# drzhn/UnitySimpleRaytracing

Measured on AMD Instinct MI355X. Metric: LBVH build Mtri/s + primary Mrays/s at 1080p on 1M-tri synthetic mesh, higher is better.
Workload: dtype f32+u32; 1 GPU; cfg2: 1,000,000-triangle tiled bumpy torus (seed 2), 1920x1080 primary rays, camera (0,0,250) fov 60; full LBVH rebuild + frame trace per step; triangles=1000000, rays=2073600, trace_mode=fast

## Files before the change

### unitysimpleraytracing_amd/csrc/lbvh_build.hip

```cpp
#include "lbvh_common.h"

namespace {

struct box3 { float mn[3]; float mx[3]; };

__device__ __forceinline__ uint32_t expand_bits(uint32_t v)
{
    v = (v * 0x00010001u) & 0xFF0000FFu;
    v = (v * 0x00000101u) & 0x0F00F00Fu;
    v = (v * 0x00000011u) & 0xC30C30C3u;
    v = (v * 0x00000005u) & 0x49249249u;
    return v;
}

__device__ __forceinline__ uint32_t quantize(float x)
{
    x = fminf(fmaxf(x * 1024.0f, 0.0f), 1023.0f);
    return (uint32_t)x;
}

struct node_reset { uint32_t* internal; uint32_t* leaf; };
__device__ __forceinline__ void reset_node_slot(const node_reset& r, uint32_t i, uint32_t n, uint32_t capacity)
{
    if (!r.internal || i >= capacity) return;
// ... 288 lines not shown

template <typename Pred>
__device__ __forceinline__ uint32_t last_true_64ary(uint32_t lo, uint32_t hi, Pred pred)
{
    const uint32_t lane = lane_id();
    while (hi - lo > 1u) {
        const uint32_t span = hi - lo;
        const uint32_t step = (span + 63u) / 64u;
        const uint32_t l = lo + (lane + 1u) * step;
        const bool p = lane < 63u && l < hi && pred(l);
        const uint64_t m = __ballot(p);
        const uint32_t cnt = (uint32_t)__builtin_ctzll(~m);
        lo += cnt * step;
        hi = min(hi, lo + step);
    }
    return lo;
}

__device__ __forceinline__ void wide_node_range(const uint32_t* __restrict__ codes, int num, int idx, uint32_t self, int d, int dmin,
                                                int& first, int& last)
{
    const uint32_t lane = lane_id();
    auto dlt = [&](int y) -> int { return (y >= 0 && y <= num - 1) ? clz32(self ^ codes[y]) : -1; };
    uint32_t lmax;
    {
        const uint32_t cand = 2u << (lane & 31u);
        const bool p = lane < 31u && dlt(idx + (int)(cand * (uint32_t)d)) > dmin;
        const uint64_t m = __ballot(p);
        lmax = 2u << (uint32_t)__builtin_ctzll(~m);
    }
    const uint32_t l = last_true_64ary(0u, lmax, [&](uint32_t q) { return dlt(idx + (int)(q * (uint32_t)d)) > dmin; });
    const int j = idx + (int)l * d;
    first = min(idx, j);
    last = max(idx, j);
}

__device__ __forceinline__ int wide_node_split(const uint32_t* __restrict__ codes, int first, int last, uint32_t first_code,
                                               uint32_t last_code)
{
    if (first_code == last_code) return (first + last) >> 1;
    const int common_prefix = clz32(first_code ^ last_code);
    return (int)last_true_64ary((uint32_t)first, (uint32_t)last,
                                [&](uint32_t q) { return clz32(first_code ^ codes[q]) > common_prefix; });
}

constexpr int kTreeWords = kTreeWindow / 32;
constexpr int kBitStride = 33;
constexpr int kBitWords = (kTreeWords + 2) * kBitStride;
constexpr int kBitSums = 34;
static_assert(kTreeHalo >= 1 && kTreeWords == (kTreeThreads + 2 * kTreeHalo) / 32 && kTreeWords <= 32,
              "the window of kTreeThreads + 2 * kTreeHalo keys needs a halo, and one 32-bit summary word per B[v]: at most 1024 keys");

template <int J>
__device__ __forceinline__ uint32_t swizzle_xor(uint32_t x)
{
    return (uint32_t)__builtin_amdgcn_ds_swizzle((int)x, (J << 10) | 0x1F);
}

template <int S>
__device__ __forceinline__ uint32_t transpose_step(uint32_t x, uint32_t keep, uint32_t amt)
{
    constexpr uint32_t J = 1u << S;
    const uint32_t y = S == 0   ? (uint32_t)__builtin_amdgcn_update_dpp(0, (int)x, 0xB1, 0xf, 0xf, true)
                       : S == 1 ? (uint32_t)__builtin_amdgcn_update_dpp(0, (int)x, 0x4E, 0xf, 0xf, true)
                                : swizzle_xor<(int)J>(x);
    const uint32_t moved = __builtin_amdgcn_alignbit(y, y, amt);
    return (x & keep) | (moved & ~keep);
}

struct transpose_consts { uint32_t keep[5], amt[5]; };
__device__ __forceinline__ transpose_consts make_transpose_consts(uint32_t lane)
{
    transpose_consts c;
    const uint32_t M[5] = {0x55555555u, 0x33333333u, 0x0F0F0F0Fu, 0x00FF00FFu, 0x0000FFFFu};
#pragma unroll
    for (int s = 0; s < 5; s++) {
        const bool upper = (lane >> s) & 1u;
        c.keep[s] = upper ? ~M[s] : M[s];
        c.amt[s] = upper ? (1u << s) : 32u - (1u << s);
    }
    return c;
}

__device__ __forceinline__ uint32_t transpose32_lanes(uint32_t x, const transpose_consts& c)
{
    x = transpose_step<0>(x, c.keep[0], c.amt[0]);
    x = transpose_step<1>(x, c.keep[1], c.amt[1]);
    x = transpose_step<2>(x, c.keep[2], c.amt[2]);
    x = transpose_step<3>(x, c.keep[3], c.amt[3]);
    x = transpose_step<4>(x, c.keep[4], c.amt[4]);
    return x;
}

typedef __attribute__((address_space(3))) uint32_t lds_u32_rw;
struct delta_bitmaps {
    lds_u32* bits;
    lds_u32* sums;
    __device__ __forceinline__ uint32_t word(int q, int v) const { return bits[(q + 1) * kBitStride + v]; }
    __device__ __forceinline__ bool first_from(int v, int s, int& pos) const
    {
        const int q = s >> 5;
        const u64 w = (((u64)word(q + 1, v) << 32) | word(q, v)) >> (s & 31);
        if (w) { pos = s + __builtin_ctzll(w); return true; }
        const uint32_t rest = sums[v] & ~((4u << q) - 1u);
        if (!rest) return false;
        const int c = __builtin_ctz(rest);
        pos = c * 32 + __builtin_ctz(word(c, v));
        return true;
    }
    __device__ __forceinline__ bool last_upto(int v, int e, int& pos) const
    {
        if (e < 0) return false;
        const int q = e >> 5;
        const u64 w = (((u64)word(q, v) << 32) | word(q - 1, v)) << (31 - (e & 31));
        if (w) { pos = e - __builtin_clzll(w); return true; }
        const uint32_t rest = q >= 1 ? sums[v] & ((1u << (q - 1)) - 1u) : 0u;
        if (!rest) return false;
        const int c = 31 - __builtin_clz(rest);
        pos = c * 32 + 31 - __builtin_clz(word(c, v));
        return true;
    }
};

__device__ __forceinline__ void clear_delta_bitmaps(uint32_t* s_bits, uint32_t* s_sums)
{
    const uint32_t t = threadIdx.x;
    if (t < (uint32_t)kBitStride) s_bits[t] = 0u;
    else if (t < 2u * kBitStride) s_bits[(kTreeWords + 1) * kBitStride + (t - kBitStride)] = 0u;
    else if (t < 2u * kBitStride + kBitSums) s_sums[t - 2u * kBitStride] = 0u;
}

__device__ __forceinline__ void stage_keys_and_bitmaps(const uint32_t* __restrict__ codes, uint32_t* s_keys, uint32_t* s_bits,
                                                       uint32_t* s_sums, const key_window& win)
{
    const uint32_t lane = lane_id(), wave = threadIdx.x >> 6;
    constexpr int kChunks = kTreeWindow / 64, kWaves = kTreeThreads / 64, kPer = kChunks / kWaves;
    static_assert(kChunks % kWaves == 0, "every wave takes the same number of chunks");
    uint32_t key[kPer], next[kPer];
#pragma unroll
    for (int k = 0; k < kPer; k++) {
        const int m = win.w0 + ((int)wave + k * kWaves) * 64 + (int)lane;
        key[k] = m < win.w1 ? codes[m] : 0u;
        next[k] = 0u;
        if (lane == 63u && m + 1 < win.w1) next[k] = codes[m + 1];
    }
    const transpose_consts tc = make_transpose_consts(lane);
    uint32_t some = 0u;
#pragma unroll
    for (int k = 0; k < kPer; k++) {
        const int c = (int)wave + k * kWaves;
        const int p = c * 64 + (int)lane, m = win.w0 + p;
        if (m < win.w1) s_keys[p] = key[k];
        const uint32_t from_next_lane = (uint32_t)__builtin_amdgcn_update_dpp(0, (int)key[k], 0x130, 0xf, 0xf, false);
        const uint32_t nxt = lane == 63u ? next[k] : from_next_lane;
        uint32_t row = 0u;
        if (m + 1 < win.w1) {
            const uint32_t x = key[k] ^ nxt;
            row = x ? 0xFFFFFFFFu << __builtin_clz(x) : 0u;
            if (!x) s_sums[32] = 1u;
        } else if (m + 1 == win.num && m < win.w1) {
            row = 0xFFFFFFFFu;
        }
        const uint32_t x = transpose32_lanes(row, tc);
        const int wd = 2 * c + (int)(lane >> 5);
        s_bits[(wd + 1) * kBitStride + (int)(lane & 31u)] = x;
        some |= x ? 1u << wd : 0u;
    }
    if (some) atomicOr(&s_sums[lane & 31u], some);
}

typedef float f3 __attribute__((ext_vector_type(3)));
struct corner3 { float x, y, z; };
struct hier_t {
    corner3* lo;
    corner3* hi;
    uint32_t n2x2;
    uint32_t levels;
};

__device__ __forceinline__ uint32_t hier_offset(uint32_t n2x2, uint32_t k) { return n2x2 - (n2x2 >> k); }

__device__ __forceinline__ f3 load_corner(const corner3* p) { return *reinterpret_cast<const f3 __attribute__((aligned(4)))*>(p); }
__device__ __forceinline__ void store_corner(corner3* p, float x, float y, float z)
{
    f3 v = {x, y, z};
    *reinterpret_cast<f3 __attribute__((aligned(4)))*>(p) = v;
}

__device__ __forceinline__ void wave_union(float mn[3], float mx[3])
{
#pragma unroll
    for (int d = 1; d < 64; d <<= 1) {
#pragma unroll
        for (int k = 0; k < 3; k++) {
            mn[k] = fminf(mn[k], __shfl_xor(mn[k], d));
            mx[k] = fmaxf(mx[k], __shfl_xor(mx[k], d));
        }
    }
}

typedef uint32_t u3v __attribute__((ext_vector_type(3)));
template <int NQ, int LV, bool BUF>
__device__ __forceinline__ void range_boxes_impl(const hier_t& h, const uint32_t a[NQ], const uint32_t b[NQ], float mn[NQ][3],
                                                 float mx[NQ][3])
{
    const uint32_t neutral = h.n2x2 - 1u;
    __amdgpu_buffer_rsrc_t lo_rsrc, hi_rsrc;
    if (BUF) {
        lo_rsrc = __builtin_amdgcn_make_buffer_rsrc(h.lo, 0, (int)(h.n2x2 * 12u), 0x00020000);
        hi_rsrc = __builtin_amdgcn_make_buffer_rsrc(h.hi, 0, (int)(h.n2x2 * 12u), 0x00020000);
    }
    uint32_t l[NQ], r[NQ];
    bool more = false;
    f3 lo[NQ][LV][2], hi[NQ][LV][2];
#pragma unroll
    for (int q = 0; q < NQ; q++) {
        l[q] = a[q];
        r[q] = b[q] + 1u;
        more = more || l[q] < r[q];
#pragma unroll
        for (int d = 0; d < 3; d++) { mn[q][d] = INFINITY; mx[q][d] = -INFINITY; }
#pragma unroll
        for (int v = 0; v < LV; v++)
#pragma unroll
            for (int e = 0; e < 2; e++) {
                const f3 pinf = {INFINITY, INFINITY, INFINITY}, ninf = {-INFINITY, -INFINITY, -INFINITY};
                lo[q][v][e] = pinf;
                hi[q][v][e] = ninf;
            }
    }
    for (uint32_t k = 0; more; k += LV) {
        uint32_t idx[NQ][LV][2];
        more = false;
#pragma unroll
        for (int v = 0; v < LV; v++) {
            const uint32_t lev = min(k + (uint32_t)v, 31u);
            const uint32_t off = hier_offset(h.n2x2, lev);
#pragma unroll
            for (int q = 0; q < NQ; q++) {
                const bool tl = l[q] < r[q] && (l[q] & 1u);
                idx[q][v][0] = tl ? off + l[q] : neutral;
                l[q] += tl ? 1u : 0u;
                const bool tr = l[q] < r[q] && (r[q] & 1u);
                r[q] -= tr ? 1u : 0u;
                idx[q][v][1] = tr ? off + r[q] : neutral;
                l[q] >>= 1;
                r[q] >>= 1;
            }
        }
#pragma unroll
        for (int q = 0; q < NQ; q++)
#pragma unroll
            for (int v = 0; v < LV; v++)
#pragma unroll
                for (int e = 0; e < 2; e++) {
                    if (idx[q][v][e] != neutral) {
                        if (BUF) {
                            const u3v x = __builtin_amdgcn_raw_buffer_load_b96(lo_rsrc, idx[q][v][e] * 12u, 0, 0);
                            const u3v y = __builtin_amdgcn_raw_buffer_load_b96(hi_rsrc, idx[q][v][e] * 12u, 0, 0);
                            lo[q][v][e].x = __uint_as_float(x.x); lo[q][v][e].y = __uint_as_float(x.y); lo[q][v][e].z = __uint_as_float(x.z);
                            hi[q][v][e].x = __uint_as_float(y.x); hi[q][v][e].y = __uint_as_float(y.y); hi[q][v][e].z = __uint_as_float(y.z);
                        } else {
                            lo[q][v][e] = load_corner(h.lo + idx[q][v][e]);
                            hi[q][v][e] = load_corner(h.hi + idx[q][v][e]);
                        }
                    }
                }
#pragma unroll
        for (int q = 0; q < NQ; q++) {
#pragma unroll
            for (int v = 0; v < LV; v++)
#pragma unroll
                for (int e = 0; e < 2; e++) {
                    mn[q][0] = fminf(mn[q][0], lo[q][v][e].x); mn[q][1] = fminf(mn[q][1], lo[q][v][e].y);
                    mn[q][2] = fminf(mn[q][2], lo[q][v][e].z);
                    mx[q][0] = fmaxf(mx[q][0], hi[q][v][e].x); mx[q][1] = fmaxf(mx[q][1], hi[q][v][e].y);
                    mx[q][2] = fmaxf(mx[q][2], hi[q][v][e].z);
                }
            more = more || l[q] < r[q];
        }
    }
}

template <int NQ, int LV>
__device__ __forceinline__ void range_boxes(const hier_t& h, const uint32_t a[NQ], const uint32_t b[NQ], float mn[NQ][3],
                                            float mx[NQ][3])
{
    if (h.n2x2 <= 0x15555555u) range_boxes_impl<NQ, LV, true>(h, a, b, mn, mx);
    else range_boxes_impl<NQ, LV, false>(h, a, b, mn, mx);
}

#ifndef LBVH_RQ_LV1
#define LBVH_RQ_LV1 3
#endif
#ifndef LBVH_RQ_LV2
#define LBVH_RQ_LV2 3
#endif
enum { TREE_TOPOLOGY = 0, TREE_REFERENCE = 1, TREE_FUSED = 2 };
#ifdef LBVH_TREE_LOOPS
constexpr bool kTreeLookups = false;
#else
constexpr bool kTreeLookups = true;
#endif
template <int MODE, bool LOOKUPS = kTreeLookups>
__device__ __forceinline__ void tree_body(uint32_t block, uint32_t* s_keys, uint32_t* s_bits, uint32_t* s_sums, float4* s_out,
                                          const uint32_t* __restrict__ codes,
                                          uint32_t n, lbvh_internal_node* __restrict__ internal, lbvh_leaf_node* __restrict__ leaf,
                                          uint32_t* __restrict__ zero_word, hier_t hier, lbvh_aabb* __restrict__ bvh,
                                          lbvh_fast_node* __restrict__ fused, uint32_t leaf_base,
                                          const uint32_t* __restrict__ sorted_indices)
{
    const uint32_t thread_id = block * kTreeThreads + threadIdx.x;
    if (thread_id == 0 && zero_word) *zero_word = 0u;
    key_window win;
    win.lds = (lds_u32*)s_keys;
    win.num = (int)n;
    win.w0 = max((int)(block * kTreeThreads) - kTreeHalo, 0);
    win.w1 = min((int)(block * kTreeThreads) + kTreeThreads + kTreeHalo, (int)n);
    if (LOOKUPS) {
        clear_delta_bitmaps(s_bits, s_sums);
        __syncthreads();
        stage_keys_and_bitmaps(codes, s_keys, s_bits, s_sums, win);
    } else {
        for (int k = win.w0 + (int)threadIdx.x; k < win.w1; k += kTreeThreads) s_keys[k - win.w0] = codes[k];
    }
    __syncthreads();
    const bool in_range = thread_id < n - 1;
    const int idx = in_range ? (int)thread_id : win.w0;
    const uint32_t self = win.at(idx);
    bool wide = false;

    const int dl = win.delta(self, idx - 1, wide);
    const int dr = win.delta(self, idx + 1, wide);
    const int diff = dr - dl;
    const int d = (diff > 0) - (diff < 0);
    const int dmin = d > 0 ? dl : (d < 0 ? dr : clz32(0u));
    int first, last, split;
    const bool lookups = LOOKUPS && s_sums[32] == 0u;
    if (lookups) {
        const delta_bitmaps bm = {(lds_u32*)s_bits, (lds_u32*)s_sums};
        const int p0 = idx - win.w0;
        int j = idx, pos = 0;
        if (d > 0) {
            if (dmin < 0) {
                if (win.w1 == win.num) j = win.num - 1; else wide = true;
            } else if (bm.first_from(dmin, p0, pos)) {
                j = win.w0 + pos;
            } else {
                wide = true;
            }
        } else if (d < 0) {
            if (bm.last_upto(dmin, p0 - 1, pos)) j = win.w0 + pos + 1;
            else if (win.w0 == 0) j = 0;
            else wide = true;
        }
        first = min(idx, j);
        last = max(idx, j);
        split = first;
        if (!wide) {
            const uint32_t x = win.at(first) ^ win.at(last);
            if (x == 0u) split = (first + last) >> 1;
            else if (bm.first_from(__builtin_clz(x), first - win.w0, pos)) split = win.w0 + pos;
            else wide = true;
        }
    } else {
        uint32_t lmax = 2;
        while (in_range && win.delta(self, idx + (int)(lmax * (uint32_t)d), wide) > dmin) lmax *= 2;
        int l = 0;
        for (uint32_t t = lmax / 2; t >= 1 && in_range && !wide; t /= 2) {
            if (win.delta(self, idx + (int)(((uint32_t)l + t) * (uint32_t)d), wide) > dmin)
                l += (int)t;
        }
        const int j = idx + l * d;
        first = min(idx, j);
        last = max(idx, j);

        split = first;
        if (in_range && !wide) {
            if (!win.inside(first) || !win.inside(last)) {
                wide = true;
            } else {
                const uint32_t first_code = win.at(first);
                const uint32_t last_code = win.at(last);
                if (first_code == last_code) {
                    split = (first + last) >> 1;
                } else {
                    const int common_prefix = clz32(first_code ^ last_code);
                    split = first;
                    int step = last - first;
                    do {
                        step = (step + 1) >> 1;
                        const int new_split = split + step;
                        if (new_split < last) {
                            const int split_prefix = clz32(first_code ^ win.at(new_split));
                            if (split_prefix > common_prefix) split = new_split;
                        }
                    } while (step > 1);
                }
            }
        }
    }
    for (uint64_t todo = __ballot(in_range && wide); todo != 0; todo &= todo - 1) {
        const int src = __builtin_ctzll(todo);
        const int widx = __builtin_amdgcn_readlane(idx, src);
        const uint32_t wself = (uint32_t)__builtin_amdgcn_readlane((int)self, src);
        const int wd = __builtin_amdgcn_readlane(d, src), wdmin = __builtin_amdgcn_readlane(dmin, src);
        int f, la, sp;
        wide_node_range(codes, (int)n, widx, wself, wd, wdmin, f, la);
        const uint32_t other = codes[widx == f ? la : f];
        const uint32_t fc = widx == f ? wself : other, lc = widx == f ? other : wself;
        int pos = 0;
        if (lookups && fc != lc && win.inside(f) &&
            delta_bitmaps{(lds_u32*)s_bits, (lds_u32*)s_sums}.first_from(__builtin_clz(fc ^ lc), f - win.w0, pos) && win.w0 + pos < la)
            sp = win.w0 + pos;
        else
            sp = wide_node_split(codes, f, la, fc, lc);
        if ((int)lane_id() == src) { first = f; last = la; split = sp; }
    }
    const bool valid = in_range && !(split < 0 || (uint32_t)split + 1u >= n);

    const bool left_leaf = split == first;
    const bool right_leaf = split + 1 == last;
    if (MODE != TREE_FUSED && valid) {
        uint32_t* node = reinterpret_cast<uint32_t*>(&internal[thread_id]);
        typedef uint32_t u2v __attribute__((ext_vector_type(2)));
        auto st2 = [](void* p, uint32_t x, uint32_t y) {
            const u2v v = {x, y};
            if (MODE == TREE_REFERENCE) __builtin_nontemporal_store(v, reinterpret_cast<u2v*>(p));
            else *reinterpret_cast<u2v*>(p) = v;
        };
        auto st1 = [](uint32_t* p, uint32_t x) {
            if (MODE == TREE_REFERENCE) __builtin_nontemporal_store(x, p);
            else *p = x;
        };
        st2(node + 0, (uint32_t)split, left_leaf ? LBVH_LEAF_NODE : LBVH_INTERNAL_NODE);
        st2(node + 2, (uint32_t)split + 1u, right_leaf ? LBVH_LEAF_NODE : LBVH_INTERNAL_NODE);
        st1(&node[5], thread_id);
        if (left_leaf) st2(&leaf[split], thread_id, (uint32_t)split);
        else st1(&internal[split].parent, thread_id);
        if (right_leaf) st2(&leaf[split + 1], thread_id, (uint32_t)split + 1u);
        else st1(&internal[split + 1].parent, thread_id);
    }
    constexpr int kQuads = MODE == TREE_FUSED ? 4 : 2;
    if (MODE == TREE_REFERENCE) {
        const uint32_t a[1] = {(uint32_t)first}, b[1] = {valid ? (uint32_t)last : (uint32_t)first};
        float mn[1][3], mx[1][3];
        range_boxes<1, LBVH_RQ_LV1>(hier, a, b, mn, mx);
        s_out[threadIdx.x * 2 + 0] = make_float4(mn[0][0], mn[0][1], mn[0][2], 0.0f);
        s_out[threadIdx.x * 2 + 1] = make_float4(mx[0][0], mx[0][1], mx[0][2], 0.0f);
    }
    if (MODE == TREE_FUSED) {
        const uint32_t a[2] = {(uint32_t)first, (uint32_t)split + 1u};
        const uint32_t b[2] = {(uint32_t)split, valid ? (uint32_t)last : (uint32_t)split};
        float cmn[2][3], cmx[2][3];
        range_boxes<1, LBVH_RQ_LV2>(hier, &a[0], &b[0], &cmn[0], &cmx[0]);
        range_boxes<1, LBVH_RQ_LV2>(hier, &a[1], &b[1], &cmn[1], &cmx[1]);
        uint32_t lref = (uint32_t)split, rref = (uint32_t)split + 1u;
        if (valid && left_leaf) lref = 0x80000000u | (leaf_base + sorted_indices[split]);
        if (valid && right_leaf) rref = 0x80000000u | (leaf_base + sorted_indices[split + 1]);
        s_out[threadIdx.x * 4 + 0] = make_float4(cmn[0][0], cmn[0][1], cmn[0][2], __uint_as_float(lref));
        s_out[threadIdx.x * 4 + 1] = make_float4(cmx[0][0], cmx[0][1], cmx[0][2], __uint_as_float(rref));
        s_out[threadIdx.x * 4 + 2] = make_float4(cmn[1][0], cmn[1][1], cmn[1][2], __uint_as_float((uint32_t)split));
        s_out[threadIdx.x * 4 + 3] = make_float4(cmx[1][0], cmx[1][1], cmx[1][2], __uint_as_float((uint32_t)split + 1u));
    }
    if (MODE != TREE_TOPOLOGY) {
        __builtin_amdgcn_fence(__ATOMIC_RELEASE, "wavefront");
        __builtin_amdgcn_wave_barrier();
        const uint32_t b0 = block * kTreeThreads;
        float4* out = MODE == TREE_FUSED ? reinterpret_cast<float4*>(fused + b0) : reinterpret_cast<float4*>(bvh + b0);
        const uint32_t live = n - 1 > b0 ? min(n - 1 - b0, (uint32_t)kTreeThreads) * kQuads : 0u;
        const uint32_t wbase = (threadIdx.x >> 6) * 64u * kQuads;
#pragma unroll
        for (int k = 0; k < kQuads; k++) {
            const uint32_t q = wbase + (uint32_t)k * 64u + lane_id();
            if (q < live) {
                if (MODE == TREE_REFERENCE) lbvh_nt_store(&out[q], s_out[q]);
                else out[q] = s_out[q];
            }
        }
    }
}

template <int MODE>
__global__ __launch_bounds__(kTreeThreads) void tree_kernel(const uint32_t* __restrict__ codes, uint32_t n,
                                                            lbvh_internal_node* __restrict__ internal,
                                                            lbvh_leaf_node* __restrict__ leaf, uint32_t* __restrict__ zero_word,
                                                            hier_t hier, lbvh_aabb* __restrict__ bvh,
                                                            lbvh_fast_node* __restrict__ fused, uint32_t leaf_base,
                                                            const uint32_t* __restrict__ sorted_indices)
{
    __shared__ uint32_t s_keys[kTreeWindow];
    __shared__ float4 s_out[MODE == TREE_TOPOLOGY ? 1 : kTreeThreads * (MODE == TREE_FUSED ? 4 : 2)];
    __shared__ uint32_t s_bits[kBitWords];
    __shared__ uint32_t s_sums[kBitSums];
    tree_body<MODE>(blockIdx.x, s_keys, s_bits, s_sums, s_out, codes, n, internal, leaf, zero_word, hier, bvh, fused, leaf_base, sorted_indices);
}

__global__ __launch_bounds__(kTreeThreads) void tree_pair_kernel(const uint32_t* __restrict__ aligned_codes,
                                                                 const uint32_t* __restrict__ codes, uint32_t n,
                                                                 lbvh_internal_node* __restrict__ internal,
                                                                 lbvh_leaf_node* __restrict__ leaf, hier_t hier,
                                                                 lbvh_aabb* __restrict__ bvh, lbvh_fast_node* __restrict__ fused,
                                                                 uint32_t leaf_base, const uint32_t* __restrict__ sorted_indices)
{
    __shared__ uint32_t s_keys[kTreeWindow];
    __shared__ float4 s_out[kTreeThreads * 4];
    __shared__ uint32_t s_bits[kBitWords];
    __shared__ uint32_t s_sums[kBitSums];
    const uint32_t block = blockIdx.x >> 1;
    if (blockIdx.x & 1u)
        tree_body<TREE_REFERENCE>(block, s_keys, s_bits, s_sums, s_out, codes, n, internal, leaf, nullptr, hier, bvh, nullptr, 0u, nullptr);
    else
        tree_body<TREE_FUSED>(block, s_keys, s_bits, s_sums, s_out, aligned_codes, n, nullptr, nullptr, nullptr, hier, nullptr, fused, leaf_base,
                              sorted_indices);
}


__device__ __forceinline__ void load_box_plain(const lbvh_aabb* p, float mn[3], float mx[3])
{
    const float4* q = reinterpret_cast<const float4*>(p);
    const float4 a = q[0], b = q[1];
    mn[0] = a.x; mn[1] = a.y; mn[2] = a.z;
    mx[0] = b.x; mx[1] = b.y; mx[2] = b.z;
}

__device__ __forceinline__ void store_box_plain(lbvh_aabb* p, const float mn[3], const float mx[3])
{
    float4* q = reinterpret_cast<float4*>(p);
    q[0] = make_float4(mn[0], mn[1], mn[2], 0.0f);
    q[1] = make_float4(mx[0], mx[1], mx[2], 0.0f);
}

constexpr int kRefitThreads = 1024;
constexpr int kLevel1Shift = 6;
constexpr int kFanShift = 4;
constexpr int kMaxLevels = 8;

struct refit_levels_t {
    lbvh_aabb* box[kMaxLevels + 1];
    uint32_t count[kMaxLevels + 1];
    int levels;
};

__global__ __launch_bounds__(kRefitThreads) void refit_kernel(uint32_t n, const lbvh_internal_node* __restrict__ internal,
                                                              const lbvh_leaf_node* __restrict__ leaf,
                                                              const lbvh_aabb* __restrict__ tri_aabb,
                                                              const uint32_t* __restrict__ sorted_indices,
                                                              lbvh_aabb* bvh, refit_levels_t lv,
                                                              uint32_t* __restrict__ frontier_count,
                                                              uint32_t* __restrict__ frontier_list)
{
    __shared__ float4 s_box[2][kRefitThreads][2];
    __shared__ uint32_t s_flag[kRefitThreads];
    __shared__ float s_wave[6][kRefitThreads / LBVH_WAVE];
    __shared__ uint2 s_node[kRefitThreads];
    __shared__ uint32_t s_front_n, s_front_base;
    const uint32_t t = threadIdx.x;
    const uint32_t b0 = blockIdx.x * (uint32_t)kRefitThreads;
    const uint32_t j = b0 + t;
    s_flag[t] = 0;
    if (t == 0) s_front_n = 0;
    if (j < n - 1) {
        const uint32_t* nd = reinterpret_cast<const uint32_t*>(&internal[j]);
        s_node[t] = make_uint2(nd[0], nd[4]);
    }
    __syncthreads();

    uint32_t q = 0xFFFFFFFFu, child_id = j, first = j, last = j;
    uint32_t child_leaf = 0x80000000u;
    float mn[3] = {INFINITY, INFINITY, INFINITY}, mx[3] = {-INFINITY, -INFINITY, -INFINITY};
    if (j < n) {
        load_box_plain(&tri_aabb[sorted_indices ? sorted_indices[j] : j], mn, mx);
        q = leaf[j].parent;
    }
    {
        float wmn[3] = {mn[0], mn[1], mn[2]}, wmx[3] = {mx[0], mx[1], mx[2]};
        wave_union(wmn, wmx);
        if ((t & 63u) == 0) {
            if ((j >> kLevel1Shift) < lv.count[1]) store_box_plain(&lv.box[1][j >> kLevel1Shift], wmn, wmx);
#pragma unroll
            for (int k = 0; k < 3; k++) { s_wave[k][t >> 6] = wmn[k]; s_wave[3 + k][t >> 6] = wmx[k]; }
        }
        __syncthreads();
        if (t < 64u) {
            float bmn[3], bmx[3];
#pragma unroll
            for (int k = 0; k < 3; k++) {
                bmn[k] = t < (uint32_t)(kRefitThreads / LBVH_WAVE) ? s_wave[k][t] : INFINITY;
                bmx[k] = t < (uint32_t)(kRefitThreads / LBVH_WAVE) ? s_wave[3 + k][t] : -INFINITY;
            }
            wave_union(bmn, bmx);
            if (t == 0 && lv.levels >= 2) store_box_plain(&lv.box[2][blockIdx.x], bmn, bmx);
        }
    }
    if (j < n) {
        for (int guard = 0; q != 0xFFFFFFFFu && guard < 64; guard++) {
            if (q >= n - 1) break;
            const bool local = q >= b0 && q - b0 < (uint32_t)kRefitThreads && first >= b0 &&
                               last - b0 < (uint32_t)kRefitThreads;
            if (!local) break;
            const uint32_t slot = q - b0;
            const uint2 nd = s_node[slot];
            const uint32_t next = nd.y;
            const uint32_t side = nd.x == child_id ? 0u : 1u;
            s_box[side][slot][0] = make_float4(mn[0], mn[1], mn[2],
                                               __uint_as_float((first - b0) | ((last - b0) << 16) | child_leaf));
            s_box[side][slot][1] = make_float4(mx[0], mx[1], mx[2], 0.0f);
            const uint32_t old = atomicAdd(&s_flag[slot], side == 0 ? 1u : 0x10000u);
            if (old == 0) break;
            const uint32_t o = side ^ 1u;
            const float4 omn = s_box[o][slot][0], omx = s_box[o][slot][1];
            const uint32_t orange = __float_as_uint(omn.w);
            mn[0] = fminf(mn[0], omn.x); mn[1] = fminf(mn[1], omn.y); mn[2] = fminf(mn[2], omn.z);
            mx[0] = fmaxf(mx[0], omx.x); mx[1] = fmaxf(mx[1], omx.y); mx[2] = fmaxf(mx[2], omx.z);
            first = min(first, b0 + (orange & 0xFFFFu));
            last = max(last, b0 + ((orange >> 16) & 0x7FFFu));
            if (q == 0) break;
            child_id = q;
            child_leaf = 0u;
            q = next;
        }
    }
    __syncthreads();
    const bool is_front = j < n - 1 && s_flag[t] != 0x10001u;
    uint32_t my = 0;
    if (is_front) my = atomicAdd(&s_front_n, 1u);
#pragma unroll
    for (uint32_t k = 0; k < 2; k++) {
        const uint32_t slot = (t >> 1) + 512u * k, h = t & 1u, node = b0 + slot;
        if (node >= n - 1 || s_flag[slot] != 0x10001u) continue;
        const float4 l = s_box[0][slot][h], r = s_box[1][slot][h];
        reinterpret_cast<float4*>(&bvh[node])[h] =
            h == 0u ? make_float4(fminf(l.x, r.x), fminf(l.y, r.y), fminf(l.z, r.z), 0.0f)
                    : make_float4(fmaxf(l.x, r.x), fmaxf(l.y, r.y), fmaxf(l.z, r.z), 0.0f);
    }
    __syncthreads();
    if (t == 0 && s_front_n)
        s_front_base = __hip_atomic_fetch_add(frontier_count, s_front_n, __ATOMIC_RELAXED, __HIP_MEMORY_SCOPE_AGENT);
    __syncthreads();
    if (is_front) frontier_list[s_front_base + my] = j;
}

__global__ __launch_bounds__(256) void refit_level_kernel(refit_levels_t lv, int k)
{
    const uint32_t e = blockIdx.x * 256u + threadIdx.x;
    if (e >= lv.count[k]) return;
    float mn[3] = {INFINITY, INFINITY, INFINITY}, mx[3] = {-INFINITY, -INFINITY, -INFINITY};
    const uint32_t c0 = e << kFanShift, c1 = min(c0 + (1u << kFanShift), lv.count[k - 1]);
    for (uint32_t c = c0; c < c1; c++) {
        float a[3], b[3];
        load_box_plain(&lv.box[k - 1][c], a, b);
#pragma unroll
        for (int d = 0; d < 3; d++) { mn[d] = fminf(mn[d], a[d]); mx[d] = fmaxf(mx[d], b[d]); }
    }
    store_box_plain(&lv.box[k][e], mn, mx);
}

__device__ __forceinline__ void node_range(uint32_t n, const lbvh_internal_node* __restrict__ internal, uint32_t p,
                                           uint32_t* first, uint32_t* last)
{
    const uint32_t* nd = reinterpret_cast<const uint32_t*>(&internal[p]);
    const bool first_kind = p <= nd[0];
    uint32_t other = first_kind ? n - 1 : 0u;
    uint32_t c = nd[4];
    if (p == 0) c = 0xFFFFFFFFu;
    for (int guard = 0; c < n - 1 && guard < 64; guard++) {
        const uint32_t* cd = reinterpret_cast<const uint32_t*>(&internal[c]);
        if ((c <= cd[0]) != first_kind) { other = c; break; }
        if (c == 0) break;
        c = cd[4];
    }
    *first = first_kind ? p : other;
    *last = first_kind ? other : p;
}

__global__ __launch_bounds__(256) void refit_frontier_kernel(uint32_t n, const lbvh_internal_node* __restrict__ internal,
                                                             const uint32_t* __restrict__ count, const uint32_t* __restrict__ list,
                                                             const lbvh_aabb* __restrict__ tri_aabb,
                                                             const uint32_t* __restrict__ sorted_indices, lbvh_aabb* bvh,
                                                             refit_levels_t lv)
{
    const uint32_t lane = lane_id();
    const uint32_t waves = gridDim.x * 4u;
    const uint32_t total = *count;
    for (uint32_t e = blockIdx.x * 4u + (threadIdx.x >> 6); e < total; e += waves) {
        const uint32_t node = list[e];
        uint32_t first, last;
        node_range(n, internal, node, &first, &last);
        if (first > last || last >= n) continue;
        float mn[3] = {INFINITY, INFINITY, INFINITY}, mx[3] = {-INFINITY, -INFINITY, -INFINITY};
        auto take = [&](const lbvh_aabb* p) {
            float a[3], b[3];
            load_box_plain(p, a, b);
#pragma unroll
            for (int d = 0; d < 3; d++) { mn[d] = fminf(mn[d], a[d]); mx[d] = fmaxf(mx[d], b[d]); }
        };
        uint32_t lo = first, hi = last + 1u;
        {
            const uint32_t a_end = min(hi, (lo + 63u) & ~63u), b_start = max(a_end, hi & ~63u);
            if (lo + lane < a_end) { const uint32_t i = lo + lane; take(&tri_aabb[sorted_indices ? sorted_indices[i] : i]); }
            if (b_start + lane < hi) { const uint32_t i = b_start + lane; take(&tri_aabb[sorted_indices ? sorted_indices[i] : i]); }
            lo = (lo + 63u) >> kLevel1Shift;
            hi >>= kLevel1Shift;
        }
        for (int k = 1; k <= lv.levels && lo < hi; k++) {
            if (k == lv.levels) {
                for (uint32_t c = lo + lane; c < hi; c += 64u) take(&lv.box[k][c]);
                break;
            }
            const uint32_t a_end = min(hi, (lo + 15u) & ~15u), b_start = max(a_end, hi & ~15u);
            if (lane < 16u) { if (lo + lane < a_end) take(&lv.box[k][lo + lane]); }
            else if (lane < 32u) { if (b_start + (lane - 16u) < hi) take(&lv.box[k][b_start + (lane - 16u)]); }
            lo = (lo + 15u) >> kFanShift;
            hi >>= kFanShift;
        }
        wave_union(mn, mx);
        if (lane == 0) store_box_plain(&bvh[node], mn, mx);
    }
}

__device__ __forceinline__ int32_t wave_inclusive_max(int32_t v)
{
#pragma unroll
    for (int d = 1; d < 64; d <<= 1) {
        const int32_t o = __shfl_up(v, d);
        if ((int)lane_id() >= d) v = max(v, o);
    }
    return v;
}

constexpr int kAkThreads = 256;

__device__ __forceinline__ int32_t block_inclusive_max(int32_t v, int32_t* s_wave, int32_t* block_max)
{
    const uint32_t t = threadIdx.x;
    const int32_t incl = wave_inclusive_max(v);
    if ((t & 63) == 63) s_wave[t >> 6] = incl;
    __syncthreads();
    int32_t prefix = INT32_MIN, all = INT32_MIN;
#pragma unroll
    for (uint32_t i = 0; i < kAkThreads / LBVH_WAVE; i++) {
        const int32_t x = s_wave[i];
        if (i < (t >> 6)) prefix = max(prefix, x);
        all = max(all, x);
    }
    *block_max = all;
    return max(incl, prefix);
}

constexpr int kAkItems = 4;
constexpr uint32_t kAkChunk = kAkThreads * kAkItems;
constexpr uint32_t kHierLocalLevels = 10;

__device__ __forceinline__ void store_hier(const hier_t& h, uint32_t k, uint32_t block, const float mn[3], const float mx[3])
{
    const size_t e = (size_t)hier_offset(h.n2x2, k) + block;
    store_corner(h.lo + e, mn[0], mn[1], mn[2]);
    store_corner(h.hi + e, mx[0], mx[1], mx[2]);
}

template <bool TERMS>
__device__ __forceinline__ void gather_hier_body(uint32_t block, const lbvh_aabb* __restrict__ tri_aabb,
                                                 const uint32_t* __restrict__ sorted_indices, uint32_t n, const box3& scene,
                                                 const hier_t& hier, int32_t* __restrict__ terms, int32_t* __restrict__ chunk_max)
{
    __shared__ int32_t s_wave[kAkThreads / LBVH_WAVE];
    __shared__ float s_six[6][kAkItems * (kAkThreads / LBVH_WAVE)];
    const uint32_t lane = lane_id(), w = threadIdx.x >> 6;
    int32_t mine = INT32_MIN;
    if (block == 0 && threadIdx.x == 0) {
        store_corner(hier.lo + (hier.n2x2 - 1u), INFINITY, INFINITY, INFINITY);
        store_corner(hier.hi + (hier.n2x2 - 1u), -INFINITY, -INFINITY, -INFINITY);
    }
#pragma unroll
    for (int k = 0; k < kAkItems; k++) {
        const uint32_t i = block * kAkChunk + (uint32_t)k * kAkThreads + threadIdx.x;
        float mn[3] = {INFINITY, INFINITY, INFINITY}, mx[3] = {-INFINITY, -INFINITY, -INFINITY};
        if (i < n) {
            const float4* src = reinterpret_cast<const float4*>(&tri_aabb[sorted_indices[i]]);
            const float4 a = src[0], b = src[1];
            mn[0] = a.x; mn[1] = a.y; mn[2] = a.z;
            mx[0] = b.x; mx[1] = b.y; mx[2] = b.z;
            store_hier(hier, 0, i, mn, mx);
            if (TERMS) {
                uint32_t q[3];
#pragma unroll
                for (int d = 0; d < 3; d++) {
                    float cen = (mn[d] + mx[d]) * 0.5f;
                    cen = cen - scene.mn[d];
                    cen = cen / (scene.mx[d] - scene.mn[d]);
                    q[d] = quantize(cen);
                }
                const int32_t term = (int32_t)(expand_bits(q[0]) * 4u + expand_bits(q[1]) * 2u + expand_bits(q[2])) - (int32_t)i;
                terms[i] = term;
                mine = max(mine, term);
            }
        }
#pragma unroll
        for (uint32_t lev = 1; lev <= 6; lev++) {
#pragma unroll
            for (int d = 0; d < 3; d++) {
                mn[d] = fminf(mn[d], __shfl_xor(mn[d], 1 << (lev - 1)));
                mx[d] = fmaxf(mx[d], __shfl_xor(mx[d], 1 << (lev - 1)));
            }
            if ((lane & ((1u << lev) - 1u)) == 0 && i < n && lev <= hier.levels) store_hier(hier, lev, i >> lev, mn, mx);
        }
        if (lane == 0) {
#pragma unroll
            for (int d = 0; d < 3; d++) { s_six[d][k * 4 + w] = mn[d]; s_six[3 + d][k * 4 + w] = mx[d]; }
        }
    }
    if (TERMS) {
        int32_t all;
        (void)block_inclusive_max(mine, s_wave, &all);
        if (threadIdx.x == 0) chunk_max[block] = all;
    } else {
// ... 500 lines not shown
```

Before: 12510 Mrays/s.

## Stage reference-mode topology writes in LDS and flush as coalesced 16-byte stores

In the reference tree mode, split, leaf flags and in-block parent and leaf-parent links are collected in shared memory instead of written straight to scattered global nodes. After a block barrier, threads flush whole node and leaf records as aligned 16-byte stores, falling back to per-word stores when a word was not set. Only children outside the block's range are still written directly to global memory. This aims to cut uncoalesced small stores in the build, at the cost of an extra barrier, more LDS per block, and byte-granular LDS flags that could conflict.

```diff
diff --git a/unitysimpleraytracing_amd/csrc/lbvh_build.hip b/unitysimpleraytracing_amd/csrc/lbvh_build.hip
--- a/unitysimpleraytracing_amd/csrc/lbvh_build.hip
+++ b/unitysimpleraytracing_amd/csrc/lbvh_build.hip
@@ -614,9 +614,55 @@
 #else
 constexpr bool kTreeLookups = true;
 #endif
+typedef __attribute__((address_space(3))) uint32_t topo_u32;
+typedef __attribute__((address_space(3))) uint8_t topo_u8;
+struct topo_stage {
+    static constexpr uint32_t kWords = kTreeThreads * 3 + kTreeThreads * 3 / 4;
+    static constexpr uint32_t kQuads = (kWords + 3) / 4;
+    static constexpr uint32_t kNodePieces = kTreeThreads * 6 / 4;
+    enum : uint32_t { OWN = 1, LEFT_LEAF = 2, RIGHT_LEAF = 4 };
+    topo_u32* split;
+    topo_u32* parent;
+    topo_u32* leaf_parent;
+    topo_u8* own;
+    topo_u8* parent_set;
+    topo_u8* leaf_set;
+    __device__ __forceinline__ static topo_stage at(uint32_t* lds)
+    {
+        topo_stage s;
+        s.split = (topo_u32*)lds;
+        s.parent = s.split + kTreeThreads;
+        s.leaf_parent = s.parent + kTreeThreads;
+        s.own = (topo_u8*)(s.leaf_parent + kTreeThreads);
+        s.parent_set = s.own + kTreeThreads;
+        s.leaf_set = s.parent_set + kTreeThreads;
+        return s;
+    }
+    __device__ __forceinline__ void clear() const
+    {
+        if (threadIdx.x < kTreeThreads / 2) reinterpret_cast<topo_u32*>(parent_set)[threadIdx.x] = 0u;
+    }
+    __device__ __forceinline__ uint32_t node_word(uint32_t w, uint32_t b0, bool& set) const
+    {
+        const uint32_t r = w / 6u, f = w - r * 6u;
+        const uint32_t o = own[r];
+        set = f == 4u ? parent_set[r] != 0 : (o & OWN) != 0u;
+        switch (f) {
+        case 0: return split[r];
+        case 1: return o & LEFT_LEAF ? LBVH_LEAF_NODE : LBVH_INTERNAL_NODE;
+        case 2: return split[r] + 1u;
+        case 3: return o & RIGHT_LEAF ? LBVH_LEAF_NODE : LBVH_INTERNAL_NODE;
+        case 4: return parent[r];
+        default: return b0 + r;
+        }
+    }
+};
+static_assert(kTreeThreads % 8 == 0 && topo_stage::kQuads <= kTreeThreads * 2, "the stage fits the half of tree_pair_kernel's s_out "
+              "that the reference's boxes leave free");
+
 template <int MODE, bool LOOKUPS = kTreeLookups>
 __device__ __forceinline__ void tree_body(uint32_t block, uint32_t* s_keys, uint32_t* s_bits, uint32_t* s_sums, float4* s_out,
-                                          const uint32_t* __restrict__ codes,
+                                          uint32_t* s_topo, const uint32_t* __restrict__ codes,
                                           uint32_t n, lbvh_internal_node* __restrict__ internal, lbvh_leaf_node* __restrict__ leaf,
                                           uint32_t* __restrict__ zero_word, hier_t hier, lbvh_aabb* __restrict__ bvh,
                                           lbvh_fast_node* __restrict__ fused, uint32_t leaf_base,
@@ -636,6 +682,7 @@
     } else {
         for (int k = win.w0 + (int)threadIdx.x; k < win.w1; k += kTreeThreads) s_keys[k - win.w0] = codes[k];
     }
+    if (MODE == TREE_REFERENCE) topo_stage::at(s_topo).clear();
     __syncthreads();
     const bool in_range = thread_id < n - 1;
     const int idx = in_range ? (int)thread_id : win.w0;
@@ -733,18 +780,25 @@
 
     const bool left_leaf = split == first;
     const bool right_leaf = split + 1 == last;
-    if (MODE != TREE_FUSED && valid) {
+    typedef uint32_t u2v __attribute__((ext_vector_type(2)));
+    typedef uint32_t u4v __attribute__((ext_vector_type(4)));
+    auto st4 = [](uint32_t* p, const u4v v) {
+        if (MODE == TREE_REFERENCE) __builtin_nontemporal_store(v, reinterpret_cast<u4v*>(p));
+        else *reinterpret_cast<u4v*>(p) = v;
+    };
+    auto st2 = [](void* p, uint32_t x, uint32_t y) {
+        const u2v v = {x, y};
+        if (MODE == TREE_REFERENCE) __builtin_nontemporal_store(v, reinterpret_cast<u2v*>(p));
+        else *reinterpret_cast<u2v*>(p) = v;
+    };
+    auto st1 = [](uint32_t* p, uint32_t x) {
+        if (MODE == TREE_REFERENCE) __builtin_nontemporal_store(x, p);
+        else *p = x;
+    };
+    constexpr bool kStaged = MODE == TREE_REFERENCE;
+    const topo_stage ts = topo_stage::at(s_topo);
+    if (MODE == TREE_TOPOLOGY && valid) {
         uint32_t* node = reinterpret_cast<uint32_t*>(&internal[thread_id]);
-        typedef uint32_t u2v __attribute__((ext_vector_type(2)));
-        auto st2 = [](void* p, uint32_t x, uint32_t y) {
-            const u2v v = {x, y};
-            if (MODE == TREE_REFERENCE) __builtin_nontemporal_store(v, reinterpret_cast<u2v*>(p));
-            else *reinterpret_cast<u2v*>(p) = v;
-        };
-        auto st1 = [](uint32_t* p, uint32_t x) {
-            if (MODE == TREE_REFERENCE) __builtin_nontemporal_store(x, p);
-            else *p = x;
-        };
         st2(node + 0, (uint32_t)split, left_leaf ? LBVH_LEAF_NODE : LBVH_INTERNAL_NODE);
         st2(node + 2, (uint32_t)split + 1u, right_leaf ? LBVH_LEAF_NODE : LBVH_INTERNAL_NODE);
         st1(&node[5], thread_id);
@@ -752,6 +806,28 @@
         else st1(&internal[split].parent, thread_id);
         if (right_leaf) st2(&leaf[split + 1], thread_id, (uint32_t)split + 1u);
         else st1(&internal[split + 1].parent, thread_id);
+    }
+    if (kStaged) {
+        const uint32_t b0 = block * kTreeThreads;
+        ts.own[threadIdx.x] = !valid ? 0u : topo_stage::OWN | (left_leaf ? topo_stage::LEFT_LEAF : 0u) |
+                                                (right_leaf ? topo_stage::RIGHT_LEAF : 0u);
+        if (valid) {
+            ts.split[threadIdx.x] = (uint32_t)split;
+#pragma unroll
+            for (int side = 0; side < 2; side++) {
+                const uint32_t child = (uint32_t)split + (uint32_t)side;
+                const uint32_t rel = child - b0;
+                const bool is_leaf = side == 0 ? left_leaf : right_leaf;
+                if (rel < (uint32_t)kTreeThreads) {
+                    if (is_leaf) { ts.leaf_parent[rel] = thread_id; ts.leaf_set[rel] = 1; }
+                    else { ts.parent[rel] = thread_id; ts.parent_set[rel] = 1; }
+                } else if (is_leaf) {
+                    st2(&leaf[child], thread_id, child);
+                } else {
+                    st1(&internal[child].parent, thread_id);
+                }
+            }
+        }
     }
     constexpr int kQuads = MODE == TREE_FUSED ? 4 : 2;
     if (MODE == TREE_REFERENCE) {
@@ -791,6 +867,43 @@
             }
         }
     }
+    if (kStaged) {
+        __syncthreads();
+        const uint32_t b0 = block * kTreeThreads;
+        uint32_t* const node_out = reinterpret_cast<uint32_t*>(internal) + (size_t)b0 * 6u;
+        uint32_t* const leaf_out = reinterpret_cast<uint32_t*>(leaf) + (size_t)b0 * 2u;
+        const bool node_lines = (reinterpret_cast<uintptr_t>(internal) & 15u) == 0u;
+        const bool leaf_lines = (reinterpret_cast<uintptr_t>(leaf) & 15u) == 0u;
+#pragma unroll
+        for (int k = 0; k < 2; k++) {
+            const uint32_t piece = (uint32_t)k * kTreeThreads + threadIdx.x;
+            u4v v;
+            bool set[4];
+            uint32_t* dst;
+            bool lines;
+            if (piece < topo_stage::kNodePieces) {
+                const uint32_t w0 = piece * 4u;
+#pragma unroll
+                for (int j = 0; j < 4; j++) v[j] = ts.node_word(w0 + (uint32_t)j, b0, set[j]);
+                dst = node_out + w0;
+                lines = node_lines;
+            } else {
+                const uint32_t l0 = (piece - topo_stage::kNodePieces) * 2u;
+                v = u4v{ts.leaf_parent[l0], b0 + l0, ts.leaf_parent[l0 + 1u], b0 + l0 + 1u};
+                set[0] = set[1] = ts.leaf_set[l0] != 0;
+                set[2] = set[3] = ts.leaf_set[l0 + 1u] != 0;
+                dst = leaf_out + l0 * 2u;
+                lines = leaf_lines;
+            }
+            if (lines && set[0] && set[1] && set[2] && set[3]) {
+                st4(dst, v);
+            } else {
+#pragma unroll
+                for (int j = 0; j < 4; j++)
+                    if (set[j]) st1(dst + j, v[j]);
+            }
+        }
+    }
 }
 
 template <int MODE>
@@ -802,10 +915,11 @@
                                                             const uint32_t* __restrict__ sorted_indices)
 {
     __shared__ uint32_t s_keys[kTreeWindow];
-    __shared__ float4 s_out[MODE == TREE_TOPOLOGY ? 1 : kTreeThreads * (MODE == TREE_FUSED ? 4 : 2)];
+    constexpr uint32_t kBoxQuads = MODE == TREE_TOPOLOGY ? 1 : kTreeThreads * (MODE == TREE_FUSED ? 4 : 2);
+    __shared__ float4 s_out[kBoxQuads + (MODE == TREE_REFERENCE ? topo_stage::kQuads : 0)];
     __shared__ uint32_t s_bits[kBitWords];
     __shared__ uint32_t s_sums[kBitSums];
-    tree_body<MODE>(blockIdx.x, s_keys, s_bits, s_sums, s_out, codes, n, internal, leaf, zero_word, hier, bvh, fused, leaf_base, sorted_indices);
+    tree_body<MODE>(blockIdx.x, s_keys, s_bits, s_sums, s_out, reinterpret_cast<uint32_t*>(s_out + kBoxQuads), codes, n, internal, leaf, zero_word, hier, bvh, fused, leaf_base, sorted_indices);
 }
 
 __global__ __launch_bounds__(kTreeThreads) void tree_pair_kernel(const uint32_t* __restrict__ aligned_codes,
@@ -821,9 +935,9 @@
     __shared__ uint32_t s_sums[kBitSums];
     const uint32_t block = blockIdx.x >> 1;
     if (blockIdx.x & 1u)
-        tree_body<TREE_REFERENCE>(block, s_keys, s_bits, s_sums, s_out, codes, n, internal, leaf, nullptr, hier, bvh, nullptr, 0u, nullptr);
+        tree_body<TREE_REFERENCE>(block, s_keys, s_bits, s_sums, s_out, reinterpret_cast<uint32_t*>(s_out + kTreeThreads * 2), codes, n, internal, leaf, nullptr, hier, bvh, nullptr, 0u, nullptr);
     else
-        tree_body<TREE_FUSED>(block, s_keys, s_bits, s_sums, s_out, aligned_codes, n, nullptr, nullptr, nullptr, hier, nullptr, fused, leaf_base,
+        tree_body<TREE_FUSED>(block, s_keys, s_bits, s_sums, s_out, nullptr, aligned_codes, n, nullptr, nullptr, nullptr, hier, nullptr, fused, leaf_base,
                               sorted_indices);
 }
 
```

Result: no change. 12490 Mrays/s (-0.2%).
